# indrajeetadityaroy9/vit-inductive-bias-distillation

Hardware: AMD Instinct MI355X
Metric: distillation images/sec (BASD loss fwd+bwd+grad all-reduce), DeiT-S<-ResNet-50 @ bs256/GPU (higher is better)
Workload: dtype f32; 1 GPU; cfg2 DeiT-S<-ResNet-50 224x224; per_gpu_batch=256, global_batch=256, input_dtype=float32, layout=strided (CLS-sliced / channel-major views), backward=True, grad_allreduce_bytes=88202672, grad_allreduce=none at world size 1 (bucket packed, nothing to exchange), rank_readback=auto, readback_deferred_steps=1756, selector=basd_selector_chain mode 0, parallelism=dp1

## Files before the change

include/basd_hip.h:

```cpp
#ifndef BASD_HIP_H
#define BASD_HIP_H

#include <stdint.h>

#ifdef __cplusplus
extern "C" {
#endif

#ifndef __HIP_PLATFORM_AMD__
typedef struct ihipStream_t* hipStream_t;
#endif

#define BASD_OK 0
#define BASD_EINVAL (-1)
#define BASD_EUNSUPPORTED (-2)
#define BASD_DTYPE_F32 0
#define BASD_DTYPE_BF16 1
#define BASD_DTYPE_U8 2


int basd_gemm_nt(const void* a, int a_dtype, long a_sb, long a_sn, long a_sd, int a_rows_per_batch,
                 long a_batch_stride, const float* b, long ldb, long b_batch_stride, int M, int N, int K, int batch,
                 float* c, long ldc, long c_batch_stride, float scale, const float* bias, float beta,
                 float* colsum_part, float* col_mean, hipStream_t stream);
// ... 200 lines not shown

int basd_gram_f64(const float* p, long p_batch_stride, int n, int D, int batch, double* g, long g_batch_stride,
                  hipStream_t stream);

int basd_gram_f64_split(const float* p, long p_batch_stride, int n, int D, int batch, int splits, double* slabs,
                        double* g, hipStream_t stream);

int basd_chol_f64(const double* g, long g_batch_stride, int n, int batch, double* l, long l_batch_stride,
                  hipStream_t stream);

int basd_stack_product(const double* la, const double* lb, long l_batch_stride, int n, int batch, int lb_period,
                       float* w, long w_batch_stride, hipStream_t stream);

int basd_procrustes_finalize(const float* w, long w_batch_stride, const float* sigma, int n, int n_s, int batch,
                             int t_period ,
                             const double* gb, long g_batch_stride, const float* omega, const int* tap0,
                             const int* tap1, const float* lam, const float* tr_s_part, int tr_slabs, float* tr_s,
                             float* tr_t, float* nuc, float* loss, float* k_prime, hipStream_t stream);

int basd_student_project_multi(const void* const* x_ptrs, int dtype, long sb, long sn, int E, int B, int n_s, int n_t,
                               int D, int ptrs_16B_aligned, const float* omega, long omega_e_stride, const int* tap0,
                               const int* tap1, const float* lam, const int* range0, const int* range1, float* mu,
                               float* tr_s, float* a_prime, hipStream_t stream);
int basd_student_grad_multi(const void* const* x_ptrs, int dtype, long sb, long sn, int E, int B, int n_s, int n_t,
                            int D, const float* omega, long omega_e_stride, const float* mu, const float* h,
                            const int* tap0, const int* tap1, const float* lam, const float* scale_ptr,
                            float scale_const, float* dx, const float* tnorm2, float* gomega, hipStream_t stream);
int basd_student_grad_fused(const void* const* x_ptrs, int dtype, long sb, long sn, int E, int B, int n_s, int n_t,
                            int D, int ptrs_16B_aligned, const float* omega, long omega_e_stride, const float* mu,
                            const float* k_prime, const float* a_prime, const int* tap0, const int* tap1,
                            const float* lam, const float* scale_ptr, float scale_const, float* dx,
                            hipStream_t stream);

typedef struct BasdProcrustesArgs {
    const void* const* student_ptrs;
    const void* const* student_host_ptrs;
    long s_dtype, s_sb, s_sn, s_aligned;
    const void* const* tok_ptrs;
    long t_dtype, t_sb, t_sn, t_sd;
    const void* const* attn_ptrs;
    long a_dtype, a_sb, a_sh, a_sq, a_sk;
    const float* mix;
    long E, L, G, B, n_s, n_t, d_s, d_t, H, A, has_cls, n_a, n, max_sweeps;
    const int* atap0; const int* atap1; const float* alam;
    const int* tap0; const int* tap1; const float* lam; const int* range0; const int* range1;
    const int* g0; const int* g1; const float* glam;
// ... 330 lines not shown
```

vit-inductive-bias-distillation_amd/basd_amd/_lib.py:

```python
from __future__ import annotations

import ctypes as C
import os
import threading

_HERE = os.path.dirname(os.path.abspath(__file__))
LIB_PATH = os.path.join(_HERE, "libbasd_hip.so")

vp, i32, i64, f32, f64 = C.c_void_p, C.c_int, C.c_long, C.c_float, C.c_double

SIGNATURES = {
    "basd_gemm_nt": [vp, i32, i64, i64, i64, i32, i64, vp, i64, i64, i32, i32, i32, i32, vp, i64, i64, f32, vp, f32,
                     vp, vp, vp],
    "basd_gemm_tn_splits": [i32],
    "basd_gemm_tn": [vp, vp, i32, i64, i64, i64, i64, i64, i64, i64, i64, i32, i32, i32, i32, i32, vp, vp, i32, vp,
                     vp, i64, i64, f32, vp],
    "basd_colmean_parts": [i32],
    "basd_colmean": [vp, i32, i64, i64, i64, i32, i64, i32, i32, i32, i32, vp, vp, vp],
    "basd_colmean_multi": [vp, i32, i64, i64, i64, i32, i32, i32, i32, i32, vp, vp, i32, vp],
    "basd_syrk_splits": [i32, i32, i32],
    "basd_syrk_multi": [vp, i32, i64, i64, i64, i32, i32, i32, i32, vp, vp, i32, vp, vp, i64, i32, vp, i32, i32, vp],
    "basd_jacobi_workspace_ints": [i32, i32],
    "basd_jacobi_max_rows": [],
    "basd_jacobi_twopass_workspace_bytes": [i32, i32, i32],
# ... 34 lines not shown
    "basd_cross_entropy": [vp, i32, i64, i32, i32, vp, vp, i64, f32, i64, vp, vp, vp],
    "basd_token_weights": [vp, i32, vp, i32, i64, i64, i64, i64, i32, i32, i32, i32, i32, i32, i32, vp, vp, vp, vp,
                           vp, vp, vp, vp, vp, vp],
    "basd_student_project": [vp, i32, i64, i64, i32, i32, i32, i32, vp, vp, vp, vp, vp, vp, vp, vp, vp, vp],
    "basd_teacher_center": [vp, i32, vp, i32, i64, i64, i64, i32, i32, i32, vp, vp, vp, vp, vp, vp, vp],
    "basd_teacher_center_multi": [vp, i32, vp, i32, i32, i64, i64, i64, i32, i32, i32, vp, vp, vp, vp, vp, vp, vp],
    "basd_teacher_center_stream_scratch_floats": [i32, i32, i32, i32],
    "basd_teacher_center_stream": [vp, i32, vp, i32, i32, i64, i64, i64, i32, i32, i32, vp, vp, vp, vp, vp, vp, vp, vp],
    "basd_gram_f64": [vp, i64, i32, i32, i32, vp, i64, vp],
    "basd_gram_f64_split": [vp, i64, i32, i32, i32, i32, vp, vp, vp],
    "basd_chol_f64": [vp, i64, i32, i32, vp, i64, vp],
    "basd_stack_product": [vp, vp, i64, i32, i32, i32, vp, i64, vp],
    "basd_procrustes_finalize": [vp, i64, vp, i32, i32, i32, i32, vp, i64, vp, vp, vp, vp, vp, i32, vp, vp, vp, vp,
                                 vp, vp],
    "basd_student_project_multi": [vp, i32, i64, i64, i32, i32, i32, i32, i32, i32, vp, i64, vp, vp, vp, vp, vp, vp,
                                   vp, vp, vp],
    "basd_student_grad_multi": [vp, i32, i64, i64, i32, i32, i32, i32, i32, vp, i64, vp, vp, vp, vp, vp, vp, f32, vp,
                                vp, vp, vp],
    "basd_student_grad_fused": [vp, i32, i64, i64, i32, i32, i32, i32, i32, i32, vp, i64, vp, vp, vp, vp, vp, vp, vp,
                                f32, vp, vp],
    "basd_procrustes_forward_fused": [vp, vp],
    "basd_procrustes_plan_query": [vp, vp],
    "basd_procrustes_tuning": [i32],
    "basd_jacobi_plain4_fits": [i32],
    "basd_stack_product_t": [vp, vp, i64, i32, i32, i32, vp, i64, vp],
    "basd_kprime_from_transposed": [vp, i64, vp, i32, i32, vp, i64, i32, vp, i64, vp, vp],
    "basd_procrustes_finish_transposed": [vp, i64, vp, i32, i32, i32, i32, vp, i64, vp, vp, vp, vp, vp, i32, vp, vp, vp,
                                          vp, vp, i64, i32, vp, vp],
    "basd_procrustes_finish_tuning": [i32],
    "basd_ustack_stash": [vp, i64, i32, i32, vp, i64, vp],
    "basd_ustack_from_transposed": [vp, i64, vp, i32, i32, vp, i64, vp, i64, vp, i32, vp, vp],
    "basd_resample_tokens": [vp, i32, i64, i64, i64, i32, i32, i32, i32, vp, vp, vp, vp, vp],
    "basd_resample_tokens_adjoint": [vp, i32, i32, i32, i32, vp, vp, vp, vp, vp, vp, vp],
    "basd_teacher_factor": [vp, i64, vp, i32, i32, i32, vp, vp, i64, vp, vp, vp, vp, vp, vp, vp, vp, vp],
    "basd_teacher_factor_tiled": [vp, i64, vp, i32, i32, i32, vp, vp, i64, vp, vp, vp, vp, vp, vp, vp, vp, vp, vp],
    "basd_mix_grad_tokens": [vp, vp, i32, i32, i64, i64, i64, i32, i32, i32, i32, vp, vp, vp, vp, vp],
    "basd_mix_grad_tokens_scratch_floats": [i32, i32, i32, i32],
    "basd_mix_grad_tokens_onepass": [vp, vp, i32, i32, i64, i64, i64, i32, i32, i32, i32, vp, vp, vp, vp, vp, vp],
    "basd_token_weight_bwd": [vp, vp, i32, i32, i32, i32, vp, vp, vp, vp, vp, vp, i32, i32, i64, i64, i64, i64, i32,
                              i32, i32, vp, vp, vp],
    "basd_build_angle_stack": [vp, i32, vp, i32, vp, vp],
    "basd_grassmann_distance_bwd": [vp, vp, i32, vp, vp, i32, vp, vp, i32, vp, vp],
    "basd_eigvec_k2": [vp, vp, i32, i32, i32, vp, vp],
    "basd_selector_chain": [vp],
    "basd_rank_certificate": [vp, vp, i32, i32, f64, vp, vp, vp],
    "basd_rank_certificate_scratch_bytes": [i32],
# ... 122 lines not shown
```

vit-inductive-bias-distillation_amd/csrc/procrustes.hip:

```cpp
#include "basd_common.h"
#include "procrustes_plan.h"

namespace basd {

typedef double f64x4 __attribute__((ext_vector_type(4)));

template <typename T>
__global__ void __launch_bounds__(256) token_weights_kernel(const void* const* __restrict__ attn_ptrs,
                                                            const float* __restrict__ mix, int L, long sb, long sh,
                                                            long sq, long sk, int H, int A, int has_cls, int n_a,
                                                            int n_t, int n_s, const int* __restrict__ atap0,
                                                            const int* __restrict__ atap1,
                                                            const float* __restrict__ alam,
                                                            const int* __restrict__ tap0,
                                                            const int* __restrict__ tap1,
                                                            const float* __restrict__ lam, float* __restrict__ omega,
                                                            float* __restrict__ omega_t, float* __restrict__ raw_out) {
    extern __shared__ float sm[];
    float* raw = sm;
    float* w = sm + n_a;
    __shared__ float red[32];
    const int b = blockIdx.x, tid = threadIdx.x;
    for (int j = tid; j < n_a; j += blockDim.x) {
        float acc = 0.f;
        if (has_cls) {
            for (int h = 0; h < H; ++h) {
                float m = 0.f;
                for (int l = 0; l < L; ++l)
                    m += mix[l] * ldg_f32((const BASD_GLOBAL_AS T*)attn_ptrs[l] + (b * sb + h * sh + (long)(1 + j) * sk));
                acc += m;
            }
            acc /= (float)H;
        } else {
            for (int h = 0; h < H; ++h)
                for (int q = 0; q < A; ++q) {
                    float m = 0.f;
                    for (int l = 0; l < L; ++l)
                        m += mix[l] * ldg_f32((const BASD_GLOBAL_AS T*)attn_ptrs[l] + (b * sb + h * sh + q * sq + (long)j * sk));
                    acc += m;
                }
            acc /= (float)(H * A);
        }
        raw[j] = acc;
        if (raw_out) raw_out[(long)b * n_a + j] = acc;
    }
    __syncthreads();
    float part = 0.f;
    for (int n = tid; n < n_s; n += blockDim.x) {
        float v;
        if (atap0) {
            const float l1 = alam[n];
            v = (1.f - l1) * raw[atap0[n]] + l1 * raw[atap1[n]];
        } else {
            v = raw[n];
        }
        w[n] = v;
        part += v;
    }
    const float total = block_sum(part, red);
    for (int n = tid; n < n_s; n += blockDim.x) {
        const float v = w[n] / total;
        w[n] = v;
        omega[(long)b * n_s + n] = v;
    }
    __syncthreads();
    for (int j = tid; j < n_t; j += blockDim.x) {
        float acc = 0.f;
        if (tap0) {
            for (int n = 0; n < n_s; ++n) {
                const float l1 = lam[n];
                if (tap0[n] == j) acc += (1.f - l1) * w[n];
                if (tap1[n] == j) acc += l1 * w[n];
            }
        } else {
            acc = w[j];
        }
        omega_t[(long)b * n_t + j] = acc;
    }
}

template <typename T>
__global__ void __launch_bounds__(256) student_project_kernel(const T* __restrict__ X, long sb, long sn, int n_s,
                                                              int n_t, int D, const float* __restrict__ omega,
                                                              const int* __restrict__ tap0,
                                                              const int* __restrict__ tap1,
                                                              const float* __restrict__ lam,
                                                              const int* __restrict__ range0,
                                                              const int* __restrict__ range1,
                                                              float* __restrict__ mu_out, float* __restrict__ tr_part,
                                                              float* __restrict__ Ap) {
    extern __shared__ float sm[];
    float* w = sm;
    __shared__ float red[4][64];
    __shared__ float mu[64];
    __shared__ float scratch[32];
    const int b = blockIdx.y, d0 = blockIdx.x * 64, tid = threadIdx.x;
    const int cl = tid & 63, rg = tid >> 6, d = d0 + cl;
    const bool live = d < D;
    const T* Xb = X + (long)b * sb + d;
    for (int n = tid; n < n_s; n += 256) w[n] = omega[(long)b * n_s + n];
// ... 17 lines not shown
            part = fmaf(w[n] * c, c, part);
        }
    const float tr = block_sum(part, scratch);
    if (tid == 0) tr_part[(long)b * gridDim.x + blockIdx.x] = tr;
    if (!live) return;
    float* Ab = Ap + (long)b * n_t * D + d;
    for (int j = rg; j < n_t; j += 4) {
        const int n0 = range0 ? range0[j] : j, n1 = range1 ? range1[j] : j + 1;
        float a = 0.f;
        for (int n = n0; n < n1; ++n) {
            float coef = 1.f;
            if (tap0) {
                const float l1 = lam[n];
                coef = (tap0[n] == j ? 1.f - l1 : 0.f) + (tap1[n] == j ? l1 : 0.f);
            }
            a = fmaf(coef * w[n], to_f32(Xb[(long)n * sn]) - m, a);
        }
        Ab[(long)j * D] = a;
    }
}

typedef float native_f32x4 __attribute__((ext_vector_type(4)));
typedef unsigned native_u32x2 __attribute__((ext_vector_type(2)));
__device__ __forceinline__ float4 ld4f(const BASD_GLOBAL_AS float* p) {
    const native_f32x4 v = *(const BASD_GLOBAL_AS native_f32x4*)p;
    return make_float4(v.x, v.y, v.z, v.w);
}
__device__ __forceinline__ float4 ld4f(const BASD_GLOBAL_AS __hip_bfloat16* p) {
    const native_u32x2 v = *(const BASD_GLOBAL_AS native_u32x2*)p;
    return make_float4(__uint_as_float(v.x << 16), __uint_as_float(v.x & 0xffff0000u), __uint_as_float(v.y << 16),
                       __uint_as_float(v.y & 0xffff0000u));
}

template <typename T>
__global__ void __launch_bounds__(256) student_project_v4_kernel(const void* const* __restrict__ x_ptrs, long sb,
                                                                 long sn, int n_s, int n_t, int D,
                                                                 const float* __restrict__ omega, long omega_e_stride,
                                                                 const int* __restrict__ tap0,
                                                                 const int* __restrict__ tap1,
                                                                 const float* __restrict__ lam,
                                                                 const int* __restrict__ range0,
                                                                 const int* __restrict__ range1,
                                                                 float* __restrict__ mu_out,
                                                                 float* __restrict__ tr_part, float* __restrict__ Ap) {
    extern __shared__ __attribute__((aligned(16))) float sm[];
    float* xs = sm;
    float* w = sm + (long)n_s * SP_W;
    float* c0 = w + n_s;
    float* c1 = c0 + n_s;
    int* t0 = (int*)(c1 + n_s);
    int* t1 = t0 + n_s;
    __shared__ __attribute__((aligned(16))) float red[32][SP_W];
    __shared__ __attribute__((aligned(16))) float mu[SP_W];
    __shared__ float scratch[32];
    const int b = blockIdx.y, e = blockIdx.z, B = gridDim.y, d0 = blockIdx.x * SP_W, tid = threadIdx.x;
    const int fq = tid & 7, rg = tid >> 3, c4 = 4 * fq;
    const bool live = d0 + c4 < D;
    const BASD_GLOBAL_AS T* Xb = (const BASD_GLOBAL_AS T*)x_ptrs[e] + (long)b * sb + d0;
    const float* om = omega + (long)e * omega_e_stride + (long)b * n_s;
    for (int n = tid; n < n_s; n += 256) {
        const float wn = om[n];
        w[n] = wn;
        if (tap0) {
            const float l1 = lam[n];
            c0[n] = (1.f - l1) * wn;
            c1[n] = l1 * wn;
            t0[n] = tap0[n];
            t1[n] = tap1[n];
        }
    }
    for (int n = rg; n < n_s; n += 32) {
        float4 v = make_float4(0.f, 0.f, 0.f, 0.f);
        if (live) v = ld4f(Xb + (long)n * sn + c4);
        *(float4*)(xs + n * SP_W + c4) = v;
    }
    __syncthreads();
    float4 acc = make_float4(0.f, 0.f, 0.f, 0.f);
    for (int n = rg; n < n_s; n += 32) {
        const float4 v = *(const float4*)(xs + n * SP_W + c4);
        const float wn = w[n];
        acc.x = fmaf(wn, v.x, acc.x); acc.y = fmaf(wn, v.y, acc.y);
        acc.z = fmaf(wn, v.z, acc.z); acc.w = fmaf(wn, v.w, acc.w);
    }
    *(float4*)(&red[rg][c4]) = acc;
    __syncthreads();
    if (tid < SP_W) {
        float m = 0.f;
#pragma unroll
        for (int q = 0; q < 32; ++q) m += red[q][tid];
        mu[tid] = m;
        if (d0 + tid < D) mu_out[((long)e * B + b) * D + d0 + tid] = m;
    }
    __syncthreads();
    const float4 m4 = *(const float4*)(mu + c4);
    float part = 0.f;
    if (live)
        for (int n = rg; n < n_s; n += 32) {
            const float4 v = *(const float4*)(xs + n * SP_W + c4);
            const float cx = v.x - m4.x, cy = v.y - m4.y, cz = v.z - m4.z, cw = v.w - m4.w;
            part = fmaf(w[n], fmaf(cx, cx, fmaf(cy, cy, fmaf(cz, cz, cw * cw))), part);
        }
    const float tr = block_sum(part, scratch);
    if (tid == 0) tr_part[((long)e * B + b) * gridDim.x + blockIdx.x] = tr;
    if (!live) return;
    float* Ab = Ap + ((long)e * B + b) * n_t * D + d0 + c4;
    for (int j = rg; j < n_t; j += 32) {
        const int n0 = range0 ? range0[j] : j, n1 = range1 ? range1[j] : j + 1;
        float4 a = make_float4(0.f, 0.f, 0.f, 0.f);
        for (int n = n0; n < n1; ++n) {
            const float cw = tap0 ? (t0[n] == j ? c0[n] : 0.f) + (t1[n] == j ? c1[n] : 0.f) : w[n];
            const float4 v = *(const float4*)(xs + n * SP_W + c4);
            a.x = fmaf(cw, v.x - m4.x, a.x); a.y = fmaf(cw, v.y - m4.y, a.y);
            a.z = fmaf(cw, v.z - m4.z, a.z); a.w = fmaf(cw, v.w - m4.w, a.w);
        }
        *(float4*)(Ab + (long)j * D) = a;
    }
}

template <typename T>
__global__ void __launch_bounds__(256) teacher_center_kernel(const void* const* __restrict__ tok_ptrs,
                                                             const float* __restrict__ mix, int L, long sb, long sn,
                                                             long sd, int n, int D, const int* __restrict__ g0,
                                                             const int* __restrict__ g1,
                                                             const float* __restrict__ glam,
                                                             const float* __restrict__ omega_t,
                                                             float* __restrict__ mu_out, float* __restrict__ Tc) {
    extern __shared__ float sm[];
    float* tile = sm;
    float* wt = sm + (size_t)n * 65;
    float* mu = wt + n;
    const int b = blockIdx.y, d0 = blockIdx.x * 64, tid = threadIdx.x;
    for (int j = tid; j < n; j += 256) wt[j] = omega_t[(long)b * n + j];
    const int total = n * 64;
    const bool feat_fast = sd == 1;
    for (int idx = tid; idx < total; idx += 256) {
        int j, dd;
        if (feat_fast) { j = idx >> 6; dd = idx & 63; }
        else { dd = idx / n; j = idx - dd * n; }
        const int d = d0 + dd;
        float v = 0.f;
        if (d < D) {
            const long off = b * sb + (long)d * sd;
            if (g0) {
                const long r0 = g0[j], r1 = g1[j];
                float a0 = 0.f, a1 = 0.f;
                for (int l = 0; l < L; ++l) {
                    const BASD_GLOBAL_AS T* p = (const BASD_GLOBAL_AS T*)tok_ptrs[l];
                    a0 = fmaf(mix[l], ldg_f32(p + (off + r0 * sn)), a0);
                    a1 = fmaf(mix[l], ldg_f32(p + (off + r1 * sn)), a1);
                }
                const float l1 = glam[j];
                v = (1.f - l1) * a0 + l1 * a1;
            } else {
                for (int l = 0; l < L; ++l)
                    v = fmaf(mix[l], ldg_f32((const BASD_GLOBAL_AS T*)tok_ptrs[l] + (off + (long)j * sn)), v);
            }
        }
        tile[j * 65 + dd] = v;
    }
    __syncthreads();
    if (tid < 64) {
        float acc = 0.f;
        for (int j = 0; j < n; ++j) acc = fmaf(wt[j], tile[j * 65 + tid], acc);
        mu[tid] = acc;
        if (d0 + tid < D) mu_out[(long)b * D + d0 + tid] = acc;
    }
    __syncthreads();
    float* out = Tc + (long)b * n * D;
    for (int idx = tid; idx < total; idx += 256) {
        const int j = idx >> 6, dd = idx & 63, d = d0 + dd;
        if (d < D) out[(long)j * D + d] = tile[j * 65 + dd] - mu[dd];
    }
}

template <typename T>
__global__ void __launch_bounds__(256) teacher_center_multi_kernel(
    const void* const* __restrict__ tok_ptrs, const float* __restrict__ mix, int L, int G, long sb, long sn, long sd,
    int n, int D, const int* __restrict__ g0, const int* __restrict__ g1, const float* __restrict__ glam,
    const float* __restrict__ omega_t, float* __restrict__ mu_out, float* __restrict__ Tc) {
    extern __shared__ float sm[];
    const int B = gridDim.y, b = blockIdx.y, d0 = blockIdx.x * TCM_W, tid = threadIdx.x;
    float* tile = sm;
    float* wt = sm + (size_t)G * n * (TCM_W + 1);
    float* mu = wt + (size_t)G * n;
    for (int idx = tid; idx < G * n; idx += 256) {
        const int g = idx / n, j = idx - g * n;
        wt[idx] = omega_t[((long)g * B + b) * n + j];
    }
    const int total = n * TCM_W;
    const bool feat_fast = sd == 1;
    for (int idx = tid; idx < total; idx += 256) {
        int j, dd;
        if (feat_fast) { j = idx / TCM_W; dd = idx - j * TCM_W; }
        else { dd = idx / n; j = idx - dd * n; }
// ... 1018 lines not shown
                                                                      const int* __restrict__ tap0,
                                                                      const int* __restrict__ tap1,
                                                                      const float* __restrict__ lam,
                                                                      const int* __restrict__ range0,
                                                                      const int* __restrict__ range1,
                                                                      float* __restrict__ dX) {
    const int j = blockIdx.x, b = blockIdx.y;
    const int s0 = range0[j], s1 = range1[j];
    for (int d = threadIdx.x; d < D; d += 128) {
        float acc = 0.f;
        for (int s = s0; s < s1; ++s) {
            const float l1 = lam[s];
            const float coef = (tap0[s] == j ? 1.f - l1 : 0.f) + (tap1[s] == j ? l1 : 0.f);
            acc = fmaf(coef, dY[((long)b * n_out + s) * D + d], acc);
        }
        dX[((long)b * n_in + j) * D + d] = acc;
    }
}

}

using namespace basd;

template <typename F>
static int with_token_type(int dtype, F&& launch) {
    if (dtype == BASD_DTYPE_F32) launch(float{});
    else if (dtype == BASD_DTYPE_BF16) launch(__hip_bfloat16{});
    else return BASD_EINVAL;
    return BASD_OK;
}

extern "C" {

int basd_token_weights(const void* const* attn_ptrs, int dtype, const float* mix, int L, long sb, long sh, long sq,
                       long sk, int B, int H, int A, int has_cls, int n_a, int n_t, int n_s, const int* atap0,
                       const int* atap1, const float* alam, const int* tap0, const int* tap1, const float* lam,
                       float* omega, float* omega_t, float* raw_out, hipStream_t stream) {
    BASD_CHECK_ARG(attn_ptrs && mix && omega && omega_t && L > 0 && B > 0 && H > 0 && n_a > 0 && n_t > 0 && n_s > 0);
    BASD_CHECK_ARG(A == n_a + (has_cls ? 1 : 0));
    BASD_CHECK_ARG((n_a == n_s) == (atap0 == nullptr));
    BASD_CHECK_ARG((n_t == n_s) == (tap0 == nullptr));
    const size_t lds = sizeof(float) * (size_t)(n_a + n_s);
    BASD_TRY(with_token_type(dtype, [&](auto t) {
        token_weights_kernel<decltype(t)><<<B, 256, lds, stream>>>(attn_ptrs, mix, L, sb, sh, sq, sk, H, A, has_cls, n_a, n_t, n_s, atap0, atap1, alam, tap0, tap1, lam, omega, omega_t, raw_out);
    }));
    BASD_RETURN_LAST();
}

int basd_student_project(const void* x, int dtype, long sb, long sn, int B, int n_s, int n_t, int D,
                         const float* omega, const int* tap0, const int* tap1, const float* lam, const int* range0,
                         const int* range1, float* mu, float* tr_s, float* a_prime, hipStream_t stream) {
    BASD_CHECK_ARG(x && omega && mu && tr_s && a_prime && B > 0 && n_s > 0 && n_t > 0 && D > 0);
    BASD_CHECK_ARG((n_t == n_s) == (tap0 == nullptr));
    const dim3 grid(plan::trace_slabs(D, SP_W1), B);
    BASD_TRY(with_token_type(dtype, [&](auto t) {
        using T = decltype(t);
        student_project_kernel<T><<<grid, 256, plan::project_lds(n_s), stream>>>((const T*)x, sb, sn, n_s, n_t, D, omega, tap0, tap1, lam, range0, range1, mu, tr_s, a_prime);
    }));
    BASD_RETURN_LAST();
}

int basd_teacher_center(const void* const* tok_ptrs, int dtype, const float* mix, int L, long sb, long sn, long sd,
                        int B, int n, int D, const int* g0, const int* g1, const float* glam, const float* omega_t,
                        float* mu, float* tc, hipStream_t stream) {
    BASD_CHECK_ARG(tok_ptrs && mix && omega_t && mu && tc && L > 0 && B > 0 && n > 0 && D > 0);
    BASD_CHECK_ARG((g0 == nullptr) == (g1 == nullptr) && (g0 == nullptr) == (glam == nullptr));
// ... 199 lines not shown
    student_grad_fused_kernel<T, RP><<<grid, 256, lds, stream>>>(x_ptrs, sb, sn, n_s, n_t, D, omega, omega_e_stride, mu, \
                                                                 k_prime, a_prime, tap0, tap1, lam, scale_ptr,      \
                                                                 scale_const, dx)
    BASD_TRY(with_token_type(dtype, [&](auto t) {
        using T = decltype(t);
        if (rp <= 4) LAUNCH_SGF(4);
        else if (rp <= 8) LAUNCH_SGF(8);
        else if (rp <= 13) LAUNCH_SGF(13);
        else LAUNCH_SGF(16);
    }));
#undef LAUNCH_SGF
    BASD_RETURN_LAST();
}

int basd_student_project_multi(const void* const* x_ptrs, int dtype, long sb, long sn, int E, int B, int n_s, int n_t,
                               int D, int ptrs_16B_aligned, const float* omega, long omega_e_stride, const int* tap0,
                               const int* tap1, const float* lam, const int* range0, const int* range1, float* mu,
                               float* tr_s, float* a_prime, hipStream_t stream) {
    BASD_CHECK_ARG(x_ptrs && omega && mu && tr_s && a_prime && E > 0 && B > 0 && n_s > 0 && n_t > 0 && D > 0);
    BASD_CHECK_ARG((n_t == n_s) == (tap0 == nullptr));
    BASD_CHECK_ARG(E <= 65535 && B <= 65535);
    if (!plan::project_multi_applies(ptrs_16B_aligned, dtype, sb, sn, D, n_s)) return BASD_EUNSUPPORTED;
    const size_t lds = plan::project_multi_lds(n_s);
    const dim3 grid(plan::trace_slabs(D, SP_W), B, E);
    BASD_TRY(with_token_type(dtype, [&](auto t) {
        using T = decltype(t);
        (void)hipFuncSetAttribute((const void*)student_project_v4_kernel<T>, hipFuncAttributeMaxDynamicSharedMemorySize, (int)lds);
        student_project_v4_kernel<T><<<grid, 256, lds, stream>>>(x_ptrs, sb, sn, n_s, n_t, D, omega, omega_e_stride, tap0, tap1, lam, range0, range1, mu, tr_s, a_prime);
    }));
    BASD_RETURN_LAST();
}

int basd_resample_tokens(const void* x, int dtype, long sb, long sn, long sd, int B, int n_in, int n_out, int D,
                         const int* tap0, const int* tap1, const float* lam, float* out, hipStream_t stream) {
    BASD_CHECK_ARG(x && tap0 && tap1 && lam && out && B > 0 && n_in > 0 && n_out > 0 && D > 0);
    const dim3 grid(n_out, B);
    BASD_TRY(with_token_type(dtype, [&](auto t) {
        using T = decltype(t);
        resample_tokens_kernel<T><<<grid, 128, 0, stream>>>((const T*)x, sb, sn, sd, n_in, n_out, D, tap0, tap1, lam, out);
    }));
    BASD_RETURN_LAST();
}

int basd_resample_tokens_adjoint(const float* dy, int B, int n_in, int n_out, int D, const int* tap0,
                                 const int* tap1, const float* lam, const int* range0, const int* range1, float* dx,
                                 hipStream_t stream) {
    BASD_CHECK_ARG(dy && tap0 && tap1 && lam && range0 && range1 && dx && B > 0 && n_in > 0 && n_out > 0 && D > 0);
    resample_tokens_adjoint_kernel<<<dim3(n_in, B), 128, 0, stream>>>(dy, n_in, n_out, D, tap0, tap1, lam, range0, range1, dx);
    BASD_RETURN_LAST();
}

}
```

vit-inductive-bias-distillation_amd/csrc/procrustes_plan.h:

```cpp
#pragma once
#include "basd_common.h"
#include "../../include/basd_hip.h"

namespace basd {

constexpr int SP_W = 32;
constexpr int SP_W1 = 64;
constexpr int TCM_W = 16, TCM_G = 4;
constexpr int TCS_ROWS = 16;
constexpr int G64_BK = 32, G64_LD = 36, G64_TPW = 8;
constexpr int CB_NB = 16, CB_KC = 64, CB_MAXR = 16;
constexpr int SG_W = 64;
constexpr int SG_LD = SG_W + 4;

namespace plan {

inline bool aligned16(const void* p) { return ((uintptr_t)p & 15) == 0; }

inline bool rows_are_quads(int dtype, long sb, long sn, int D) {
    const int esz = dtype == BASD_DTYPE_F32 ? 4 : 2;
    return D % 4 == 0 && (sb * esz) % 16 == 0 && (sn * esz) % 16 == 0 && (esz == 4 || D % 8 == 0);
}

inline size_t center_lds(int n) { return sizeof(float) * ((size_t)n * 65 + n + 64); }
inline bool center_fits(int n) { return center_lds(n) <= 150 * 1024; }
inline size_t center_multi_lds(int G, int n) {
    return sizeof(float) * ((size_t)G * n * (TCM_W + 1) + (size_t)G * n + (size_t)G * TCM_W);
}
inline bool center_multi_applies(int G, int n) { return G <= TCM_G && center_multi_lds(G, n) <= 150 * 1024; }
inline int stream_chunks(int n) { return (n + TCS_ROWS - 1) / TCS_ROWS; }
inline long stream_scratch_floats(int G, int B, int n, int D) { return (long)stream_chunks(n) * G * B * D; }
inline bool stream_applies(int G, long sd, int B) { return G <= TCM_G && sd == 1 && B <= 65535 && (long)G * B <= 65535; }
inline bool stream_v4_applies(int dtype, bool gathered, long sb, long sn, int D, const void* tc, const void* scratch) {
    return dtype == BASD_DTYPE_F32 && !gathered && D % 4 == 0 && sb % 4 == 0 && sn % 4 == 0 && aligned16(tc) &&
           aligned16(scratch);
}

inline size_t project_lds(int n_s) { return sizeof(float) * (size_t)n_s; }
inline size_t project_multi_lds(int n_s) { return sizeof(float) * ((size_t)n_s * SP_W + 5 * (size_t)n_s); }
inline bool project_multi_applies(int ptrs_aligned, int dtype, long sb, long sn, int D, int n_s) {
    return ptrs_aligned && rows_are_quads(dtype, sb, sn, D) && project_multi_lds(n_s) <= 96 * 1024;
}
inline int trace_slabs(int D, int width) { return (D + width - 1) / width; }

// ... 114 lines not shown
```

Measured before the change: 176,000 images/s.

## Parallelize token weights, persistent prefetching student projection, vectorize teacher centering

Token-weight kernel now splits the head/query reduction across thread partitions with LDS partials. It also replaces the O(n_t*n_s) tap scatter with per-target index ranges built by atomics. The student projection becomes a persistent grid-stride kernel templated on rows-per-thread: it keeps rows in registers, prefetches the next item, and reduces with DPP/permlane cross-lane ops. Teacher centering gains vectorized loads, a split mean reduction and float4 stores. These add LDS usage, register pressure and occupancy-query overhead per launch.

Result: slower. 163,000 images/s (-7.4%).

```diff
diff --git a/include/basd_hip.h b/include/basd_hip.h
--- a/include/basd_hip.h
+++ b/include/basd_hip.h
@@ -246,6 +246,7 @@
                                int D, int ptrs_16B_aligned, const float* omega, long omega_e_stride, const int* tap0,
                                const int* tap1, const float* lam, const int* range0, const int* range1, float* mu,
                                float* tr_s, float* a_prime, hipStream_t stream);
+int basd_procrustes_project_grid(int max_workgroups);
 int basd_student_grad_multi(const void* const* x_ptrs, int dtype, long sb, long sn, int E, int B, int n_s, int n_t,
                             int D, const float* omega, long omega_e_stride, const float* mu, const float* h,
                             const int* tap0, const int* tap1, const float* lam, const float* scale_ptr,
diff --git a/vit-inductive-bias-distillation_amd/basd_amd/_lib.py b/vit-inductive-bias-distillation_amd/basd_amd/_lib.py
--- a/vit-inductive-bias-distillation_amd/basd_amd/_lib.py
+++ b/vit-inductive-bias-distillation_amd/basd_amd/_lib.py
@@ -80,6 +80,7 @@
     "basd_procrustes_forward_fused": [vp, vp],
     "basd_procrustes_plan_query": [vp, vp],
     "basd_procrustes_tuning": [i32],
+    "basd_procrustes_project_grid": [i32],
     "basd_jacobi_plain4_fits": [i32],
     "basd_stack_product_t": [vp, vp, i64, i32, i32, i32, vp, i64, vp],
     "basd_kprime_from_transposed": [vp, i64, vp, i32, i32, vp, i64, i32, vp, i64, vp, vp],
diff --git a/vit-inductive-bias-distillation_amd/csrc/procrustes.hip b/vit-inductive-bias-distillation_amd/csrc/procrustes.hip
--- a/vit-inductive-bias-distillation_amd/csrc/procrustes.hip
+++ b/vit-inductive-bias-distillation_amd/csrc/procrustes.hip
@@ -19,33 +19,54 @@
     extern __shared__ float sm[];
     float* raw = sm;
     float* w = sm + n_a;
+    float* part = w + n_s;
+    float* c0 = part + TW_PART;
+    float* c1 = c0 + n_s;
+    int* t0 = (int*)(c1 + n_s);
+    int* t1 = t0 + n_s;
+    int* rlo = t1 + n_s;
+    int* rhi = rlo + n_t;
     __shared__ float red[32];
     const int b = blockIdx.x, tid = threadIdx.x;
-    for (int j = tid; j < n_a; j += blockDim.x) {
+    const int Aq = has_cls ? 1 : A, terms = H * Aq;
+    const int P = n_a <= TW_PART ? min(TW_PART / n_a, terms) : 1;
+    const int chunk = (terms + P - 1) / P;
+    const BASD_GLOBAL_AS T* a0 = (const BASD_GLOBAL_AS T*)attn_ptrs[0] + (b * sb + (long)has_cls * sk);
+    const float mix0 = mix[0];
+    for (int item = tid; item < P * n_a; item += 256) {
+        const int p = item / n_a, j = item - p * n_a;
+        const int first = p * chunk, last = min(terms, first + chunk);
+        int h = first / Aq, q = first - h * Aq;
+        long off = h * sh + q * sq + (long)j * sk;
         float acc = 0.f;
-        if (has_cls) {
-            for (int h = 0; h < H; ++h) {
-                float m = 0.f;
-                for (int l = 0; l < L; ++l)
-                    m += mix[l] * ldg_f32((const BASD_GLOBAL_AS T*)attn_ptrs[l] + (b * sb + h * sh + (long)(1 + j) * sk));
-                acc += m;
-            }
-            acc /= (float)H;
-        } else {
-            for (int h = 0; h < H; ++h)
-                for (int q = 0; q < A; ++q) {
-                    float m = 0.f;
-                    for (int l = 0; l < L; ++l)
-                        m += mix[l] * ldg_f32((const BASD_GLOBAL_AS T*)attn_ptrs[l] + (b * sb + h * sh + q * sq + (long)j * sk));
-                    acc += m;
-                }
-            acc /= (float)(H * A);
-        }
-        raw[j] = acc;
-        if (raw_out) raw_out[(long)b * n_a + j] = acc;
-    }
-    __syncthreads();
-    float part = 0.f;
+#pragma unroll 4
+        for (int t = first; t < last; ++t) {
+            float m = mix0 * ldg_f32(a0 + off);
+            for (int l = 1; l < L; ++l)
+                m += mix[l] * ldg_f32((const BASD_GLOBAL_AS T*)attn_ptrs[l] + (b * sb + (long)has_cls * sk + off));
+            acc += m;
+            off += sq;
+            if (++q == Aq) { q = 0; off += sh - Aq * sq; }
+        }
+        if (P > 1) part[item] = acc;
+        else {
+            acc /= (float)terms;
+            raw[j] = acc;
+            if (raw_out) raw_out[(long)b * n_a + j] = acc;
+        }
+    }
+    if (tap0)
+        for (int j = tid; j < n_t; j += 256) { rlo[j] = n_s; rhi[j] = -1; }
+    __syncthreads();
+    if (P > 1 && tid < n_a) {
+        float acc = part[tid];
+        for (int p = 1; p < P; ++p) acc += part[p * n_a + tid];
+        acc /= (float)terms;
+        raw[tid] = acc;
+        if (raw_out) raw_out[(long)b * n_a + tid] = acc;
+    }
+    __syncthreads();
+    float psum = 0.f;
     for (int n = tid; n < n_s; n += blockDim.x) {
         float v;
         if (atap0) {
@@ -55,27 +76,47 @@
             v = raw[n];
         }
         w[n] = v;
-        part += v;
-    }
-    const float total = block_sum(part, red);
+        psum += v;
+    }
+    const float total = block_sum(psum, red);
     for (int n = tid; n < n_s; n += blockDim.x) {
         const float v = w[n] / total;
         w[n] = v;
         omega[(long)b * n_s + n] = v;
-    }
-    __syncthreads();
-    for (int j = tid; j < n_t; j += blockDim.x) {
+        if (tap0) {
+            const float l1 = lam[n];
+            const int j0 = tap0[n], j1 = tap1[n];
+            c0[n] = (1.f - l1) * v;
+            c1[n] = l1 * v;
+            t0[n] = j0;
+            t1[n] = j1;
+            atomicMin(&rlo[j0], n); atomicMax(&rhi[j0], n);
+            atomicMin(&rlo[j1], n); atomicMax(&rhi[j1], n);
+        }
+    }
+    __syncthreads();
+    if (!tap0) {
+        for (int j = tid; j < n_t; j += 256) omega_t[(long)b * n_t + j] = w[j];
+        return;
+    }
+    const int P3 = n_t <= TW_PART ? TW_PART / n_t : 1;
+    for (int item = tid; item < P3 * n_t; item += 256) {
+        const int p = item / n_t, j = item - p * n_t;
+        const int hi = rhi[j];
         float acc = 0.f;
-        if (tap0) {
-            for (int n = 0; n < n_s; ++n) {
-                const float l1 = lam[n];
-                if (tap0[n] == j) acc += (1.f - l1) * w[n];
-                if (tap1[n] == j) acc += l1 * w[n];
-            }
-        } else {
-            acc = w[j];
-        }
-        omega_t[(long)b * n_t + j] = acc;
+        for (int n = rlo[j] + p; n <= hi; n += P3) {
+            if (t0[n] == j) acc += c0[n];
+            if (t1[n] == j) acc += c1[n];
+        }
+        if (P3 > 1) part[item] = acc;
+        else omega_t[(long)b * n_t + j] = acc;
+    }
+    if (P3 == 1) return;
+    __syncthreads();
+    if (tid < n_t) {
+        float acc = part[tid];
+        for (int p = 1; p < P3; ++p) acc += part[p * n_t + tid];
+        omega_t[(long)b * n_t + tid] = acc;
     }
 }
 
@@ -139,6 +180,7 @@
 
 typedef float native_f32x4 __attribute__((ext_vector_type(4)));
 typedef unsigned native_u32x2 __attribute__((ext_vector_type(2)));
+typedef unsigned native_u32x4 __attribute__((ext_vector_type(4)));
 __device__ __forceinline__ float4 ld4f(const BASD_GLOBAL_AS float* p) {
     const native_f32x4 v = *(const BASD_GLOBAL_AS native_f32x4*)p;
     return make_float4(v.x, v.y, v.z, v.w);
@@ -150,16 +192,41 @@
 }
 
 template <typename T>
-__global__ void __launch_bounds__(256) student_project_v4_kernel(const void* const* __restrict__ x_ptrs, long sb,
-                                                                 long sn, int n_s, int n_t, int D,
-                                                                 const float* __restrict__ omega, long omega_e_stride,
-                                                                 const int* __restrict__ tap0,
-                                                                 const int* __restrict__ tap1,
-                                                                 const float* __restrict__ lam,
-                                                                 const int* __restrict__ range0,
-                                                                 const int* __restrict__ range1,
-                                                                 float* __restrict__ mu_out,
-                                                                 float* __restrict__ tr_part, float* __restrict__ Ap) {
+struct RawQuad;
+template <>
+struct RawQuad<float> {
+    native_f32x4 r;
+    __device__ __forceinline__ void load(const BASD_GLOBAL_AS float* p) { r = *(const BASD_GLOBAL_AS native_f32x4*)p; }
+    __device__ __forceinline__ float4 get() const { return make_float4(r.x, r.y, r.z, r.w); }
+};
+template <>
+struct RawQuad<__hip_bfloat16> {
+    native_u32x2 r;
+    __device__ __forceinline__ void load(const BASD_GLOBAL_AS __hip_bfloat16* p) {
+        r = *(const BASD_GLOBAL_AS native_u32x2*)p;
+    }
+    __device__ __forceinline__ float4 get() const {
+        return make_float4(__uint_as_float(r.x << 16), __uint_as_float(r.x & 0xffff0000u), __uint_as_float(r.y << 16),
+                           __uint_as_float(r.y & 0xffff0000u));
+    }
+};
+
+__device__ __forceinline__ float rowgroups8_allsum(float x) {
+    x += dpp_get<0x128>(x);
+    auto r = __builtin_amdgcn_permlane16_swap(__float_as_uint(x), __float_as_uint(x), false, false);
+    x = __uint_as_float(r[0]) + __uint_as_float(r[1]);
+    auto q = __builtin_amdgcn_permlane32_swap(__float_as_uint(x), __float_as_uint(x), false, false);
+    return __uint_as_float(q[0]) + __uint_as_float(q[1]);
+}
+
+template <typename T, int R>
+__global__ void __launch_bounds__(256, R <= 8 ? 3 : 1)
+student_project_v4_kernel(const void* const* __restrict__ x_ptrs, long sb, long sn, int n_s, int n_t, int D, int B,
+                          int slabs, long items, const float* __restrict__ omega, long omega_e_stride,
+                          const int* __restrict__ tap0, const int* __restrict__ tap1, const float* __restrict__ lam,
+                          const int* __restrict__ range0, const int* __restrict__ range1, float* __restrict__ mu_out,
+                          float* __restrict__ tr_part, float* __restrict__ Ap) {
+    constexpr bool EARLY = R <= 8;
     extern __shared__ __attribute__((aligned(16))) float sm[];
     float* xs = sm;
     float* w = sm + (long)n_s * SP_W;
@@ -167,72 +234,148 @@
     float* c1 = c0 + n_s;
     int* t0 = (int*)(c1 + n_s);
     int* t1 = t0 + n_s;
-    __shared__ __attribute__((aligned(16))) float red[32][SP_W];
-    __shared__ __attribute__((aligned(16))) float mu[SP_W];
-    __shared__ float scratch[32];
-    const int b = blockIdx.y, e = blockIdx.z, B = gridDim.y, d0 = blockIdx.x * SP_W, tid = threadIdx.x;
-    const int fq = tid & 7, rg = tid >> 3, c4 = 4 * fq;
-    const bool live = d0 + c4 < D;
-    const BASD_GLOBAL_AS T* Xb = (const BASD_GLOBAL_AS T*)x_ptrs[e] + (long)b * sb + d0;
-    const float* om = omega + (long)e * omega_e_stride + (long)b * n_s;
-    for (int n = tid; n < n_s; n += 256) {
-        const float wn = om[n];
-        w[n] = wn;
-        if (tap0) {
-            const float l1 = lam[n];
-            c0[n] = (1.f - l1) * wn;
-            c1[n] = l1 * wn;
+    __shared__ __attribute__((aligned(16))) float red[4][SP_W];
+    __shared__ float scratch[4];
+    const int tid = threadIdx.x, fq = tid & 7, rg = tid >> 3, c4 = 4 * fq, wave = tid >> 6;
+    constexpr int Q = (32 * R + 255) / 256;
+    auto opaque_n_s = [&]() {
+        int ns = n_s;
+        asm volatile("" : "+s"(ns));
+        return ns;
+    };
+    int* rng = (int*)w;
+    const bool rng_lds = tap0 && range0;
+    if (tap0)
+        for (int n = tid; n < n_s; n += 256) {
             t0[n] = tap0[n];
             t1[n] = tap1[n];
-        }
-    }
-    for (int n = rg; n < n_s; n += 32) {
-        float4 v = make_float4(0.f, 0.f, 0.f, 0.f);
-        if (live) v = ld4f(Xb + (long)n * sn + c4);
-        *(float4*)(xs + n * SP_W + c4) = v;
-    }
-    __syncthreads();
-    float4 acc = make_float4(0.f, 0.f, 0.f, 0.f);
-    for (int n = rg; n < n_s; n += 32) {
-        const float4 v = *(const float4*)(xs + n * SP_W + c4);
-        const float wn = w[n];
-        acc.x = fmaf(wn, v.x, acc.x); acc.y = fmaf(wn, v.y, acc.y);
-        acc.z = fmaf(wn, v.z, acc.z); acc.w = fmaf(wn, v.w, acc.w);
-    }
-    *(float4*)(&red[rg][c4]) = acc;
-    __syncthreads();
-    if (tid < SP_W) {
-        float m = 0.f;
-#pragma unroll
-        for (int q = 0; q < 32; ++q) m += red[q][tid];
-        mu[tid] = m;
-        if (d0 + tid < D) mu_out[((long)e * B + b) * D + d0 + tid] = m;
-    }
-    __syncthreads();
-    const float4 m4 = *(const float4*)(mu + c4);
-    float part = 0.f;
-    if (live)
-        for (int n = rg; n < n_s; n += 32) {
-            const float4 v = *(const float4*)(xs + n * SP_W + c4);
+            if (range0 && n < n_t) rng[n] = range0[n] | range1[n] << 16;
+        }
+    float lq[Q];
+#pragma unroll
+    for (int q = 0; q < Q; ++q) lq[q] = tap0 ? lam[min(tid + 256 * q, n_s - 1)] : 0.f;
+    RawQuad<T> cur[R], nxt[EARLY ? R : 1];
+    float wr[R], wn[EARLY ? R : 1], wq[Q], wqn[EARLY ? Q : 1];
+    auto fetch = [&](long item, RawQuad<T>* x, float* wx, float* wqx) {
+        const int slab = (int)(item % slabs);
+        const long eb = item / slabs;
+        const int b = (int)(eb % B), e = (int)(eb / B), d0 = slab * SP_W;
+        const bool live = d0 + c4 < D;
+        const BASD_GLOBAL_AS T* Xb = (const BASD_GLOBAL_AS T*)x_ptrs[e] + (long)b * sb + d0 + (live ? c4 : 0);
+        const float* om = omega + (long)e * omega_e_stride + (long)b * n_s;
+        const int ns = opaque_n_s();
+#pragma unroll
+        for (int k = 0; k < R; ++k) {
+            const int n = rg + 32 * k, nc = min(n, ns - 1);
+            x[k].load(Xb + (long)nc * sn);
+            const float wk = om[nc];
+            wx[k] = n < ns ? wk : 0.f;
+        }
+#pragma unroll
+        for (int q = 0; q < Q; ++q) wqx[q] = om[min(tid + 256 * q, n_s - 1)];
+    };
+    long item = blockIdx.x;
+    if (item < items) fetch(item, cur, wr, wq);
+    for (; item < items; item += gridDim.x) {
+        const long next = item + gridDim.x;
+        if (EARLY && next < items) fetch(next, nxt, wn, wqn);
+        const int slab = (int)(item % slabs), d0 = slab * SP_W;
+        const long eb = item / slabs;
+        const bool live = d0 + c4 < D;
+        const int ns = opaque_n_s();
+        float4 acc = make_float4(0.f, 0.f, 0.f, 0.f);
+#pragma unroll
+        for (int k = 0; k < R; ++k) {
+            const float4 v = cur[k].get();
+            const float wk = wr[k];
+            acc.x = fmaf(wk, v.x, acc.x); acc.y = fmaf(wk, v.y, acc.y);
+            acc.z = fmaf(wk, v.z, acc.z); acc.w = fmaf(wk, v.w, acc.w);
+            *(float4*)(xs + min(rg + 32 * k, ns - 1) * SP_W + c4) = v;
+        }
+#pragma unroll
+        for (int q = 0; q < Q; ++q) {
+            const int n = tid + 256 * q;
+            if (n < n_s) {
+                if (tap0) { c0[n] = (1.f - lq[q]) * wq[q]; c1[n] = lq[q] * wq[q]; }
+                else w[n] = wq[q];
+            }
+        }
+        acc.x = rowgroups8_allsum(acc.x); acc.y = rowgroups8_allsum(acc.y);
+        acc.z = rowgroups8_allsum(acc.z); acc.w = rowgroups8_allsum(acc.w);
+        if (rg == 8 * wave) *(float4*)(&red[wave][c4]) = acc;
+        __syncthreads();
+        float4 m4;
+        {
+            const float4 p0 = *(const float4*)(&red[0][c4]), p1 = *(const float4*)(&red[1][c4]);
+            const float4 p2 = *(const float4*)(&red[2][c4]), p3 = *(const float4*)(&red[3][c4]);
+            m4 = make_float4((p0.x + p1.x) + (p2.x + p3.x), (p0.y + p1.y) + (p2.y + p3.y),
+                             (p0.z + p1.z) + (p2.z + p3.z), (p0.w + p1.w) + (p2.w + p3.w));
+        }
+        if (rg == 0 && live) {
+            float* mo = mu_out + eb * D + d0 + c4;
+            mo[0] = m4.x; mo[1] = m4.y; mo[2] = m4.z; mo[3] = m4.w;
+        }
+        float part = 0.f;
+#pragma unroll
+        for (int k = 0; k < R; ++k) {
+            const float4 v = cur[k].get();
             const float cx = v.x - m4.x, cy = v.y - m4.y, cz = v.z - m4.z, cw = v.w - m4.w;
-            part = fmaf(w[n], fmaf(cx, cx, fmaf(cy, cy, fmaf(cz, cz, cw * cw))), part);
-        }
-    const float tr = block_sum(part, scratch);
-    if (tid == 0) tr_part[((long)e * B + b) * gridDim.x + blockIdx.x] = tr;
-    if (!live) return;
-    float* Ab = Ap + ((long)e * B + b) * n_t * D + d0 + c4;
-    for (int j = rg; j < n_t; j += 32) {
-        const int n0 = range0 ? range0[j] : j, n1 = range1 ? range1[j] : j + 1;
-        float4 a = make_float4(0.f, 0.f, 0.f, 0.f);
-        for (int n = n0; n < n1; ++n) {
-            const float cw = tap0 ? (t0[n] == j ? c0[n] : 0.f) + (t1[n] == j ? c1[n] : 0.f) : w[n];
-            const float4 v = *(const float4*)(xs + n * SP_W + c4);
-            a.x = fmaf(cw, v.x - m4.x, a.x); a.y = fmaf(cw, v.y - m4.y, a.y);
-            a.z = fmaf(cw, v.z - m4.z, a.z); a.w = fmaf(cw, v.w - m4.w, a.w);
-        }
-        *(float4*)(Ab + (long)j * D) = a;
-    }
-}
+            part = fmaf(wr[k], fmaf(cx, cx, fmaf(cy, cy, fmaf(cz, cz, cw * cw))), part);
+        }
+        part = wave_sum(live ? part : 0.f);
+        if ((tid & 63) == 0) scratch[wave] = part;
+        if (!EARLY && next < items) fetch(next, cur, wr, wq);
+        if (live) {
+            float* Ab = Ap + eb * n_t * D + d0 + c4;
+            auto project = [&](int j, int n0, int n1) {
+                float4 a = make_float4(0.f, 0.f, 0.f, 0.f);
+                for (int n = n0; n < n1; ++n) {
+                    const float cw = tap0 ? (t0[n] == j ? c0[n] : 0.f) + (t1[n] == j ? c1[n] : 0.f) : w[n];
+                    const float4 v = *(const float4*)(xs + n * SP_W + c4);
+                    a.x = fmaf(cw, v.x - m4.x, a.x); a.y = fmaf(cw, v.y - m4.y, a.y);
+                    a.z = fmaf(cw, v.z - m4.z, a.z); a.w = fmaf(cw, v.w - m4.w, a.w);
+                }
+                *(float4*)(Ab + (long)j * D) = a;
+            };
+            for (int j = rg; j < n_t; j += 32) {
+                if (rng_lds && j < n_s) project(j, rng[j] & 0xffff, rng[j] >> 16);
+                else project(j, range0 ? range0[j] : j, range1 ? range1[j] : j + 1);
+            }
+        }
+        __syncthreads();
+        if (tid == 0) tr_part[item] = (scratch[0] + scratch[1]) + (scratch[2] + scratch[3]);
+        if (EARLY) {
+#pragma unroll
+            for (int k = 0; k < R; ++k) { cur[k] = nxt[k]; wr[k] = wn[k]; }
+#pragma unroll
+            for (int q = 0; q < Q; ++q) wq[q] = wqn[q];
+        }
+    }
+}
+
+template <typename T>
+struct TokVec;
+template <>
+struct TokVec<float> {
+    static constexpr int N = 4;
+    static __device__ __forceinline__ void load(const BASD_GLOBAL_AS float* p, float (&v)[4]) {
+        const native_f32x4 x = *(const BASD_GLOBAL_AS native_f32x4*)p;
+        v[0] = x.x; v[1] = x.y; v[2] = x.z; v[3] = x.w;
+    }
+};
+template <>
+struct TokVec<__hip_bfloat16> {
+    static constexpr int N = 8;
+    static __device__ __forceinline__ void load(const BASD_GLOBAL_AS __hip_bfloat16* p, float (&v)[8]) {
+        const native_u32x4 x = *(const BASD_GLOBAL_AS native_u32x4*)p;
+        const unsigned u[4] = {x.x, x.y, x.z, x.w};
+#pragma unroll
+        for (int i = 0; i < 4; ++i) {
+            v[2 * i] = __uint_as_float(u[i] << 16);
+            v[2 * i + 1] = __uint_as_float(u[i] & 0xffff0000u);
+        }
+    }
+};
 
 template <typename T>
 __global__ void __launch_bounds__(256) teacher_center_kernel(const void* const* __restrict__ tok_ptrs,
@@ -242,51 +385,168 @@
                                                              const float* __restrict__ glam,
                                                              const float* __restrict__ omega_t,
                                                              float* __restrict__ mu_out, float* __restrict__ Tc) {
+    constexpr int V = TokVec<T>::N;
     extern __shared__ float sm[];
     float* tile = sm;
     float* wt = sm + (size_t)n * 65;
     float* mu = wt + n;
+    __shared__ float red[4][64];
     const int b = blockIdx.y, d0 = blockIdx.x * 64, tid = threadIdx.x;
     for (int j = tid; j < n; j += 256) wt[j] = omega_t[(long)b * n + j];
     const int total = n * 64;
-    const bool feat_fast = sd == 1;
-    for (int idx = tid; idx < total; idx += 256) {
-        int j, dd;
-        if (feat_fast) { j = idx >> 6; dd = idx & 63; }
-        else { dd = idx / n; j = idx - dd * n; }
-        const int d = d0 + dd;
-        float v = 0.f;
-        if (d < D) {
-            const long off = b * sb + (long)d * sd;
+    const int feats = min(64, D - d0);
+    const long tile_off = b * sb + (long)d0 * sd;
+    const uintptr_t base0 = (uintptr_t)tok_ptrs[0];
+    bool same_offset = true, aligned = (base0 & 15) == 0;
+    for (int l = 1; l < L; ++l) {
+        const uintptr_t p = (uintptr_t)tok_ptrs[l];
+        same_offset = same_offset && ((p - base0) & 15) == 0;
+        aligned = aligned && (p & 15) == 0;
+    }
+    if (!g0 && sn == 1 && sd == n && n > 1 && same_offset) {
+        const int count = feats * n;
+        const unsigned magic = 0xFFFFFFFFu / (unsigned)n + 1u;
+        const uintptr_t addr = base0 + sizeof(T) * (uintptr_t)tile_off;
+        const int head = min(count, (int)(((16 - (addr & 15)) & 15) / sizeof(T)));
+        const int nvec = (count - head) / V, tail = head + nvec * V;
+        for (int v0 = tid; v0 < nvec; v0 += 4 * 256) {
+            float x[4][V];
+#pragma unroll
+            for (int u = 0; u < 4; ++u) {
+                const int v = v0 + u * 256;
+#pragma unroll
+                for (int e = 0; e < V; ++e) x[u][e] = 0.f;
+                if (v < nvec)
+                    for (int l = 0; l < L; ++l) {
+                        float y[V];
+                        TokVec<T>::load((const BASD_GLOBAL_AS T*)tok_ptrs[l] + (tile_off + head + (long)v * V), y);
+                        const float m = mix[l];
+#pragma unroll
+                        for (int e = 0; e < V; ++e) x[u][e] = fmaf(m, y[e], x[u][e]);
+                    }
+            }
+#pragma unroll
+            for (int u = 0; u < 4; ++u) {
+                const int v = v0 + u * 256;
+                if (v < nvec) {
+                    const int i = head + v * V;
+                    int dd = (int)__umulhi((unsigned)i, magic), j = i - dd * n;
+#pragma unroll
+                    for (int e = 0; e < V; ++e) {
+                        tile[j * 65 + dd] = x[u][e];
+                        if (++j == n) { j = 0; ++dd; }
+                    }
+                }
+            }
+        }
+        const int loose = head + (count - tail);
+        if (tid < loose) {
+            const int i = tid < head ? tid : tail + (tid - head);
+            const int dd = (int)__umulhi((unsigned)i, magic), j = i - dd * n;
+            float v = 0.f;
+            for (int l = 0; l < L; ++l)
+                v = fmaf(mix[l], ldg_f32((const BASD_GLOBAL_AS T*)tok_ptrs[l] + (tile_off + i)), v);
+            tile[j * 65 + dd] = v;
+        }
+    } else if (sd == 1 && aligned && (sb * sizeof(T)) % 16 == 0 && (sn * sizeof(T)) % 16 == 0) {
+        constexpr int PPR = 64 / V;
+        for (int idx = tid; idx < n * PPR; idx += 256) {
+            const int j = idx / PPR, dd = (idx - j * PPR) * V;
+            float x[V], x1[V];
+#pragma unroll
+            for (int e = 0; e < V; ++e) x[e] = x1[e] = 0.f;
+            const long r0 = g0 ? g0[j] : j, r1 = g0 ? g1[j] : j;
+            if (dd + V <= feats) {
+                for (int l = 0; l < L; ++l) {
+                    const BASD_GLOBAL_AS T* p = (const BASD_GLOBAL_AS T*)tok_ptrs[l] + (tile_off + dd);
+                    const float m = mix[l];
+                    float y[V];
+                    TokVec<T>::load(p + r0 * sn, y);
+#pragma unroll
+                    for (int e = 0; e < V; ++e) x[e] = fmaf(m, y[e], x[e]);
+                    if (g0) {
+                        TokVec<T>::load(p + r1 * sn, y);
+#pragma unroll
+                        for (int e = 0; e < V; ++e) x1[e] = fmaf(m, y[e], x1[e]);
+                    }
+                }
+            } else {
+                for (int l = 0; l < L; ++l) {
+                    const BASD_GLOBAL_AS T* p = (const BASD_GLOBAL_AS T*)tok_ptrs[l] + (tile_off + dd);
+                    const float m = mix[l];
+#pragma unroll
+                    for (int e = 0; e < V; ++e)
+                        if (dd + e < feats) {
+                            x[e] = fmaf(m, ldg_f32(p + (r0 * sn + e)), x[e]);
+                            if (g0) x1[e] = fmaf(m, ldg_f32(p + (r1 * sn + e)), x1[e]);
+                        }
+                }
+            }
             if (g0) {
-                const long r0 = g0[j], r1 = g1[j];
-                float a0 = 0.f, a1 = 0.f;
-                for (int l = 0; l < L; ++l) {
-                    const BASD_GLOBAL_AS T* p = (const BASD_GLOBAL_AS T*)tok_ptrs[l];
-                    a0 = fmaf(mix[l], ldg_f32(p + (off + r0 * sn)), a0);
-                    a1 = fmaf(mix[l], ldg_f32(p + (off + r1 * sn)), a1);
+                const float l1 = glam[j];
+#pragma unroll
+                for (int e = 0; e < V; ++e) x[e] = (1.f - l1) * x[e] + l1 * x1[e];
+            }
+#pragma unroll
+            for (int e = 0; e < V; ++e) tile[j * 65 + dd + e] = x[e];
+        }
+    } else {
+        const bool feat_fast = sd == 1;
+        for (int idx = tid; idx < total; idx += 256) {
+            int j, dd;
+            if (feat_fast) { j = idx >> 6; dd = idx & 63; }
+            else { dd = idx / n; j = idx - dd * n; }
+            float v = 0.f;
+            if (dd < feats) {
+                const long off = tile_off + (long)dd * sd;
+                if (g0) {
+                    const long r0 = g0[j], r1 = g1[j];
+                    float a0 = 0.f, a1 = 0.f;
+                    for (int l = 0; l < L; ++l) {
+                        const BASD_GLOBAL_AS T* p = (const BASD_GLOBAL_AS T*)tok_ptrs[l];
+                        a0 = fmaf(mix[l], ldg_f32(p + (off + r0 * sn)), a0);
+                        a1 = fmaf(mix[l], ldg_f32(p + (off + r1 * sn)), a1);
+                    }
+                    const float l1 = glam[j];
+                    v = (1.f - l1) * a0 + l1 * a1;
+                } else {
+                    for (int l = 0; l < L; ++l)
+                        v = fmaf(mix[l], ldg_f32((const BASD_GLOBAL_AS T*)tok_ptrs[l] + (off + (long)j * sn)), v);
                 }
-                const float l1 = glam[j];
-                v = (1.f - l1) * a0 + l1 * a1;
-            } else {
-                for (int l = 0; l < L; ++l)
-                    v = fmaf(mix[l], ldg_f32((const BASD_GLOBAL_AS T*)tok_ptrs[l] + (off + (long)j * sn)), v);
-            }
-        }
-        tile[j * 65 + dd] = v;
+            }
+            tile[j * 65 + dd] = v;
+        }
+    }
+    __syncthreads();
+    {
+        const int dd = tid & 63, p = tid >> 6;
+        float acc = 0.f;
+#pragma unroll 4
+        for (int j = p; j < n; j += 4) acc = fmaf(wt[j], tile[j * 65 + dd], acc);
+        red[p][dd] = acc;
     }
     __syncthreads();
     if (tid < 64) {
-        float acc = 0.f;
-        for (int j = 0; j < n; ++j) acc = fmaf(wt[j], tile[j * 65 + tid], acc);
+        const float acc = (red[0][tid] + red[1][tid]) + (red[2][tid] + red[3][tid]);
         mu[tid] = acc;
-        if (d0 + tid < D) mu_out[(long)b * D + d0 + tid] = acc;
-    }
-    __syncthreads();
-    float* out = Tc + (long)b * n * D;
-    for (int idx = tid; idx < total; idx += 256) {
-        const int j = idx >> 6, dd = idx & 63, d = d0 + dd;
-        if (d < D) out[(long)j * D + d] = tile[j * 65 + dd] - mu[dd];
+        if (tid < feats) mu_out[(long)b * D + d0 + tid] = acc;
+    }
+    __syncthreads();
+    float* out = Tc + (long)b * n * D + d0;
+    if (D % 4 == 0 && ((uintptr_t)Tc & 15) == 0) {
+        for (int idx = tid; idx < n * 16; idx += 256) {
+            const int j = idx >> 4, dd = (idx & 15) * 4;
+            if (dd < feats) {
+                const float* t = tile + j * 65 + dd;
+                *(float4*)(out + (long)j * D + dd) =
+                    make_float4(t[0] - mu[dd], t[1] - mu[dd + 1], t[2] - mu[dd + 2], t[3] - mu[dd + 3]);
+            }
+        }
+    } else {
+        for (int idx = tid; idx < total; idx += 256) {
+            const int j = idx >> 6, dd = idx & 63;
+            if (dd < feats) out[(long)j * D + dd] = tile[j * 65 + dd] - mu[dd];
+        }
     }
 }
 
@@ -1351,6 +1611,8 @@
 
 using namespace basd;
 
+static int g_project_grid = 0;
+
 template <typename F>
 static int with_token_type(int dtype, F&& launch) {
     if (dtype == BASD_DTYPE_F32) launch(float{});
@@ -1369,8 +1631,10 @@
     BASD_CHECK_ARG(A == n_a + (has_cls ? 1 : 0));
     BASD_CHECK_ARG((n_a == n_s) == (atap0 == nullptr));
     BASD_CHECK_ARG((n_t == n_s) == (tap0 == nullptr));
-    const size_t lds = sizeof(float) * (size_t)(n_a + n_s);
+    const size_t lds = plan::token_weights_lds(n_a, n_t, n_s, tap0 != nullptr);
     BASD_TRY(with_token_type(dtype, [&](auto t) {
+        if (lds > 48 * 1024)
+            (void)hipFuncSetAttribute((const void*)token_weights_kernel<decltype(t)>, hipFuncAttributeMaxDynamicSharedMemorySize, (int)lds);
         token_weights_kernel<decltype(t)><<<B, 256, lds, stream>>>(attn_ptrs, mix, L, sb, sh, sq, sk, H, A, has_cls, n_a, n_t, n_s, atap0, atap1, alam, tap0, tap1, lam, omega, omega_t, raw_out);
     }));
     BASD_RETURN_LAST();
@@ -1616,13 +1880,34 @@
     BASD_CHECK_ARG(E <= 65535 && B <= 65535);
     if (!plan::project_multi_applies(ptrs_16B_aligned, dtype, sb, sn, D, n_s)) return BASD_EUNSUPPORTED;
     const size_t lds = plan::project_multi_lds(n_s);
-    const dim3 grid(plan::trace_slabs(D, SP_W), B, E);
+    const int slabs = plan::trace_slabs(D, SP_W);
+    const long items = (long)slabs * B * E;
     BASD_TRY(with_token_type(dtype, [&](auto t) {
         using T = decltype(t);
-        (void)hipFuncSetAttribute((const void*)student_project_v4_kernel<T>, hipFuncAttributeMaxDynamicSharedMemorySize, (int)lds);
-        student_project_v4_kernel<T><<<grid, 256, lds, stream>>>(x_ptrs, sb, sn, n_s, n_t, D, omega, omega_e_stride, tap0, tap1, lam, range0, range1, mu, tr_s, a_prime);
+        auto launch = [&](auto* kernel) {
+            (void)hipFuncSetAttribute((const void*)kernel, hipFuncAttributeMaxDynamicSharedMemorySize, (int)lds);
+            int dev = 0, cus = 0, per_cu = 0;
+            if (hipGetDevice(&dev) != hipSuccess ||
+                hipDeviceGetAttribute(&cus, hipDeviceAttributeMultiprocessorCount, dev) != hipSuccess || cus <= 0)
+                cus = 256;
+            if (hipOccupancyMaxActiveBlocksPerMultiprocessor(&per_cu, (const void*)kernel, 256, lds) != hipSuccess || per_cu <= 0)
+                per_cu = 1;
+            long grid = (long)cus * per_cu;
+            if (g_project_grid > 0 && grid > g_project_grid) grid = g_project_grid;
+            if (grid > items) grid = items;
+            kernel<<<(unsigned)grid, 256, lds, stream>>>(x_ptrs, sb, sn, n_s, n_t, D, B, slabs, items, omega, omega_e_stride, tap0, tap1, lam, range0, range1, mu, tr_s, a_prime);
+        };
+        if (n_s <= 32 * SP_R_SMALL) launch(student_project_v4_kernel<T, SP_R_SMALL>);
+        else if (n_s <= 32 * SP_R_MID) launch(student_project_v4_kernel<T, SP_R_MID>);
+        else launch(student_project_v4_kernel<T, SP_R_LARGE>);
     }));
     BASD_RETURN_LAST();
+}
+
+int basd_procrustes_project_grid(int max_workgroups) {
+    const int prev = g_project_grid;
+    if (max_workgroups >= 0) g_project_grid = max_workgroups;
+    return prev;
 }
 
 int basd_resample_tokens(const void* x, int dtype, long sb, long sn, long sd, int B, int n_in, int n_out, int D,
diff --git a/vit-inductive-bias-distillation_amd/csrc/procrustes_plan.h b/vit-inductive-bias-distillation_amd/csrc/procrustes_plan.h
--- a/vit-inductive-bias-distillation_amd/csrc/procrustes_plan.h
+++ b/vit-inductive-bias-distillation_amd/csrc/procrustes_plan.h
@@ -4,7 +4,9 @@
 
 namespace basd {
 
+constexpr int TW_PART = 256;
 constexpr int SP_W = 32;
+constexpr int SP_R_SMALL = 7, SP_R_MID = 18, SP_R_LARGE = 21;
 constexpr int SP_W1 = 64;
 constexpr int TCM_W = 16, TCM_G = 4;
 constexpr int TCS_ROWS = 16;
@@ -20,6 +22,10 @@
 inline bool rows_are_quads(int dtype, long sb, long sn, int D) {
     const int esz = dtype == BASD_DTYPE_F32 ? 4 : 2;
     return D % 4 == 0 && (sb * esz) % 16 == 0 && (sn * esz) % 16 == 0 && (esz == 4 || D % 8 == 0);
+}
+
+inline size_t token_weights_lds(int n_a, int n_t, int n_s, bool taps) {
+    return sizeof(float) * ((size_t)n_a + n_s + TW_PART + (taps ? 4 * (size_t)n_s + 2 * (size_t)n_t : 0));
 }
 
 inline size_t center_lds(int n) { return sizeof(float) * ((size_t)n * 65 + n + 64); }
```
